# zyddnys/sd_animation_optical_flow

Hardware: AMD Instinct MI355X
Metric: frame-pairs/sec (flow+warp+mask) at 512x768 (higher is better)
Workload: dtype f32

## Files before the change

### sd_animation_optical_flow_amd/csrc/conv_wino.hip

```cpp
#include "ofx_internal.h"

#include <cmath>
#include <cstdlib>
#include <cstring>

namespace {

constexpr int kWBK = 16;
constexpr int kLDV = kWBK + 4;
constexpr int kOOB = 0x7FFFFFF0;

template <int W_, int H_, int LDH, int Y0, int X0> struct Halo {
    static constexpr int W = W_, H = H_, ldh = LDH, y_org = Y0, x_org = X0;
    static constexpr int pix = W * H;
    static constexpr int items = pix * (kWBK / 4);
    static constexpr int slots = (items + 255) / 256;
    static constexpr int floats = pix * ldh;
};
using Halo3x3 = Halo<18, 10, 24, -1, -1>;
template <bool VERT> using Halo15 = Halo<VERT ? 16 : 20, VERT ? 12 : 8, VERT ? 16 : 20, VERT ? -2 : 0, VERT ? 0 : -2>;

struct WinoK {
    const float* in0;
    const float* in1;
    const float* u;
    const float* scale;
    const float* shift;
    const float* addend;
    const float* res;
    const float* nmean;
    const float* nrstd;
    float* stats;
    float* out;
    float* aux_z;
    float* aux_rh;
    float* aux_h;
    int ld0, c0, ld1, cin, ldo, ldadd, ldh, ldres;
    int H, W, Cout, act;
    int nblk;
    int nb32;
    int tpr, tpi, mtiles;
    int bytes0, bytes1, bytesu;
    float alpha;
};

struct Patch {
    int nb, pb, y0, x0;
};

__device__ __forceinline__ Patch wino_patch(const WinoK& p) {
    const int nblk = p.mtiles * p.nblk;
    const int bid = blockIdx.x;
    const int q8 = nblk >> 3, r8 = nblk & 7;
    const int xcd = bid & 7, idx = bid >> 3;
    const int L = (xcd < r8 ? xcd * (q8 + 1) : r8 * (q8 + 1) + (xcd - r8) * q8) + idx;
    const int nb = L % p.nblk, mt = L / p.nblk;
    const int pb = mt / p.tpi;
    const int trem = mt - pb * p.tpi;
    const int py = trem / p.tpr;
    return {nb, pb, py * 8, (trem - py * p.tpr) * 16};
}

template <class ALG, bool NORM = false>
__device__ __forceinline__ void wino_slabs(const WinoK& p, const Patch& pt, float* Hs, float* Vs, int tid, int wave,
                                           f32x16 (&acc)[ALG::P][ALG::NT]) {
    typedef int v4i __attribute__((ext_vector_type(4)));
    using HALO = typename ALG::HALO;
    constexpr int P = ALG::P, NT = ALG::NT;
    const int lane = tid & 63;

    const float* in1s = p.in1 ? p.in1 : p.in0;
    const int bytes1s = p.in1 ? p.bytes1 : p.bytes0;
    int hpix[HALO::slots];
    unsigned hok = 0;
#pragma unroll
    for (int k = 0; k < HALO::slots; ++k) {
        const int i = tid + 256 * k;
        const int pix = i >> 2;
        const int hy = pix / HALO::W, hx = pix - hy * HALO::W;
        const int gy = pt.y0 + HALO::y_org + hy, gx = pt.x0 + HALO::x_org + hx;
        const bool ok = i < HALO::items && (unsigned)gy < (unsigned)p.H && (unsigned)gx < (unsigned)p.W;
        hpix[k] = ok ? (pt.pb * p.H + gy) * p.W + gx : 0;
        hok |= (ok ? 1u : 0u) << k;
    }
    const int hq = (tid & 3) * 16;
    float4 pa[HALO::slots];
    float4 pmu, prs;
    auto a_issue = [&](int cb) __attribute__((always_inline)) {
        const int c = cb * kWBK;
        const bool s0 = c < p.c0;
        const __amdgpu_buffer_rsrc_t rs = __builtin_amdgcn_make_buffer_rsrc((void*)(s0 ? p.in0 : in1s), (short)0, s0 ? p.bytes0 : bytes1s, 0x00020000);
        const int so = (s0 ? c : c - p.c0) * 4;
        const int ldb = (s0 ? p.ld0 : p.ld1) * 4;
#pragma unroll
        for (int k = 0; k < HALO::slots; ++k) {
            const int vo = ((hok >> k) & 1u) ? hpix[k] * ldb + hq : kOOB;
            v4i t = __builtin_amdgcn_raw_buffer_load_b128(rs, vo, so, 0);
            pa[k] = *reinterpret_cast<float4*>(&t);
        }
        if constexpr (NORM) {
            const long at = (long)pt.pb * p.c0 + c + (tid & 3) * 4;
            pmu = *reinterpret_cast<const float4*>(p.nmean + at);
            prs = *reinterpret_cast<const float4*>(p.nrstd + at);
        }
    };

    const __amdgpu_buffer_rsrc_t rsu = __builtin_amdgcn_make_buffer_rsrc((void*)p.u, (short)0, p.bytesu, 0x00020000);
    const int c8n = p.cin >> 3;
    const int wlane = lane * 16;
    const int pt0 = ALG::pt0(wave), blk0 = ALG::blk0(pt.nb, wave);
    float4 wr[P][NT][2];
    auto w_issue = [&](int q, int cb) __attribute__((always_inline)) {
#pragma unroll
        for (int nt = 0; nt < NT; ++nt)
#pragma unroll
            for (int ks = 0; ks < 2; ++ks) {
                const int so = (((pt0 + q) * p.nb32 + blk0 + nt) * c8n + 2 * cb + ks) * 1024;
                v4i t = __builtin_amdgcn_raw_buffer_load_b128(rsu, wlane, so, 0);
                wr[q][nt][ks] = *reinterpret_cast<float4*>(&t);
            }
    };

#pragma unroll
    for (int q = 0; q < P; ++q)
#pragma unroll
        for (int nt = 0; nt < NT; ++nt)
#pragma unroll
            for (int e = 0; e < 16; ++e) acc[q][nt][e] = 0.f;

    const ALG xf(Hs, Vs, tid, wave);
    const float* const afrag = Vs + (pt0 * 32 + (lane & 31)) * kLDV + 4 * (lane >> 5);

    const int CB = p.cin / kWBK;
    a_issue(0);
#pragma unroll
    for (int q = 0; q < P; ++q) w_issue(q, 0);
    for (int cb = 0; cb < CB; ++cb) {
        const int nx = cb + 1 < CB ? cb + 1 : cb;
#pragma unroll
        for (int k = 0; k < HALO::slots; ++k) {
            const int i = tid + 256 * k;
            if (HALO::slots * 256 > HALO::items && k == HALO::slots - 1 && i >= HALO::items) break;
            float4 v = pa[k];
            if constexpr (NORM) {
                v.x = fmaxf((v.x - pmu.x) * prs.x, 0.f);
                v.y = fmaxf((v.y - pmu.y) * prs.y, 0.f);
                v.z = fmaxf((v.z - pmu.z) * prs.z, 0.f);
                v.w = fmaxf((v.w - pmu.w) * prs.w, 0.f);
                if (!((hok >> k) & 1u)) v = make_float4(0.f, 0.f, 0.f, 0.f);
            }
            *reinterpret_cast<float4*>(&Hs[(i >> 2) * HALO::ldh + (i & 3) * 4]) = v;
        }
        __syncthreads();
        xf();
        __syncthreads();
        a_issue(nx);
        __builtin_amdgcn_sched_barrier(0);
#pragma unroll
        for (int q = 0; q < P; ++q) {
#pragma unroll
            for (int ks = 0; ks < 2; ++ks) {
                const float4 a = *reinterpret_cast<const float4*>(afrag + q * 32 * kLDV + 8 * ks);
#pragma unroll
                for (int nt = 0; nt < NT; ++nt) {
                    const float4 b = wr[q][nt][ks];
                    acc[q][nt] = __builtin_amdgcn_mfma_f32_32x32x2f32(a.x, b.x, acc[q][nt], 0, 0, 0);
                    acc[q][nt] = __builtin_amdgcn_mfma_f32_32x32x2f32(a.y, b.y, acc[q][nt], 0, 0, 0);
                    acc[q][nt] = __builtin_amdgcn_mfma_f32_32x32x2f32(a.z, b.z, acc[q][nt], 0, 0, 0);
                    acc[q][nt] = __builtin_amdgcn_mfma_f32_32x32x2f32(a.w, b.w, acc[q][nt], 0, 0, 0);
                }
            }
            w_issue(q, nx);
        }
    }
}

__device__ __forceinline__ float2 f2(float a, float b) { return make_float2(a, b); }
__device__ __forceinline__ float2 operator+(float2 a, float2 b) { return f2(a.x + b.x, a.y + b.y); }
__device__ __forceinline__ float2 operator-(float2 a, float2 b) { return f2(a.x - b.x, a.y - b.y); }
__device__ __forceinline__ float2 operator*(float s, float2 a) { return f2(s * a.x, s * a.y); }

struct Wino3x3 {
    using HALO = Halo3x3;
    static constexpr int P = 4, NT = 2;
    __device__ static int pt0(int wave) { return 4 * wave; }
    __device__ static int blk0(int nb, int) { return 2 * nb; }
    const float* src;
    float* dst;
    __device__ __forceinline__ Wino3x3(const float* Hs, float* Vs, int tid, int wave) {
        const int ttx = (tid & 63) >> 3, tcp = tid & 7;
        src = Hs + (2 * wave * HALO::W + 2 * ttx) * HALO::ldh + 2 * tcp;
        dst = Vs + (wave * 8 + ttx) * kLDV + 2 * tcp;
    }
    __device__ __forceinline__ void operator()() const {
        float2 d[4][4];
#pragma unroll
        for (int r = 0; r < 4; ++r)
#pragma unroll
            for (int c = 0; c < 4; ++c) d[r][c] = *reinterpret_cast<const float2*>(src + (r * HALO::W + c) * HALO::ldh);
        float2 t[4][4];
#pragma unroll
        for (int c = 0; c < 4; ++c) {
            t[0][c] = d[0][c] - d[2][c];
            t[1][c] = d[1][c] + d[2][c];
            t[2][c] = d[2][c] - d[1][c];
            t[3][c] = d[1][c] - d[3][c];
        }
#pragma unroll
        for (int i = 0; i < 4; ++i) {
            float2 v[4];
            v[0] = t[i][0] - t[i][2];
            v[1] = t[i][1] + t[i][2];
            v[2] = t[i][2] - t[i][1];
            v[3] = t[i][1] - t[i][3];
#pragma unroll
            for (int j = 0; j < 4; ++j) *reinterpret_cast<float2*>(dst + (i * 4 + j) * 32 * kLDV) = v[j];
        }
    }
};

template <bool VERT> struct Wino15 {
    using HALO = Halo15<VERT>;
    static constexpr int P = 8, NT = 1;
    __device__ static int pt0(int) { return 0; }
    __device__ static int blk0(int nb, int wave) { return 4 * nb + wave; }
    static constexpr int tap = (VERT ? HALO::W : 1) * HALO::ldh;
    const float* src;
    float* dst;
    __device__ static int base(int t) { return VERT ? (4 * (t >> 4)) * HALO::W + (t & 15) : (t >> 2) * HALO::W + 4 * (t & 3); }
    __device__ static int oy(int t, int i) { return VERT ? 4 * (t >> 4) + i : t >> 2; }
    __device__ static int ox(int t, int i) { return VERT ? (t & 15) : 4 * (t & 3) + i; }
    __device__ __forceinline__ Wino15(const float* Hs, float* Vs, int tid, int) {
        const int ttile = tid >> 3, tcp = tid & 7;
        src = Hs + base(ttile) * HALO::ldh + 2 * tcp;
        dst = Vs + ttile * kLDV + 2 * tcp;
    }
    __device__ __forceinline__ void operator()() const {
        float2 d[8];
#pragma unroll
        for (int j = 0; j < 8; ++j) d[j] = *reinterpret_cast<const float2*>(src + j * tap);
        float2 v[8];
        v[0] = (d[0] - d[6]) + 5.25f * (d[4] - d[2]);
        v[7] = (d[7] - d[1]) + 5.25f * (d[3] - d[5]);
        float2 te = (d[2] + d[6]) - 4.25f * d[4], to = (d[1] + d[5]) - 4.25f * d[3];
        v[1] = te + to;
        v[2] = te - to;
        te = (0.25f * d[2] + d[6]) - 1.25f * d[4];
        to = (0.5f * d[1] - 2.5f * d[3]) + 2.0f * d[5];
        v[3] = te + to;
        v[4] = te - to;
        te = (4.0f * d[2] + d[6]) - 5.0f * d[4];
        to = (2.0f * d[1] - 2.5f * d[3]) + 0.5f * d[5];
        v[5] = te + to;
        v[6] = te - to;
#pragma unroll
        for (int j = 0; j < 8; ++j) *reinterpret_cast<float2*>(dst + j * 32 * kLDV) = v[j];
    }
};

constexpr int kLDX = 32;
constexpr int kVF2 = 16 * 32 * kLDV;
constexpr int kSmem2 = Halo3x3::floats + kVF2;
constexpr int kXF = 4 * 2 * 32 * kLDX;
static_assert(kXF + 2 * 4 * 32 * 2 <= kSmem2, "exchange and statistics must fit");

template <bool NORM, bool RES, bool STATS>
__global__ __launch_bounds__(256, 2) void wino_conv_kernel(const WinoK p) {
    __shared__ __attribute__((aligned(16))) float smem[kSmem2];
    float* const Hs = smem;
    float* const Vs = smem + Halo3x3::floats;
    const int tid = threadIdx.x, lane = tid & 63;
    const int wave = __builtin_amdgcn_readfirstlane(tid >> 6);
    const Patch pt = wino_patch(p);
    f32x16 acc[4][2];
    wino_slabs<Wino3x3, NORM>(p, pt, Hs, Vs, tid, wave, acc);

    const float act_lo = p.act == OFX_ACT_RELU ? 0.0f : -3.402823466e38f;
    float* const X = smem;
    float* const Sx = smem + kXF;
    const int on = tid & 31, otx = tid >> 5;
#pragma unroll
    for (int nt = 0; nt < 2; ++nt) {
        __syncthreads();
#pragma unroll
        for (int e = 0; e < 16; ++e) {
            const int tile = (e & 3) + 8 * (e >> 2) + 4 * (lane >> 5);
            const float m0 = acc[0][nt][e], m1 = acc[1][nt][e], m2 = acc[2][nt][e], m3 = acc[3][nt][e];
            X[((wave * 2 + 0) * 32 + tile) * kLDX + (lane & 31)] = m0 + m1 + m2;
            X[((wave * 2 + 1) * 32 + tile) * kLDX + (lane & 31)] = m1 - m2 - m3;
        }
        __syncthreads();
        const int oc = pt.nb * 64 + nt * 32 + on;
        if (oc < p.Cout) {
            const float sc = (p.scale ? p.scale[oc] : 1.0f) * p.alpha;
            const float sh = p.shift ? p.shift[oc] : 0.0f;
            float st_s = 0.0f, st_q = 0.0f;
#pragma unroll
            for (int ty = 0; ty < 4; ++ty) {
                const int tile = ty * 8 + otx;
                float x[4][2];
#pragma unroll
                for (int w = 0; w < 4; ++w)
#pragma unroll
                    for (int j = 0; j < 2; ++j) x[w][j] = X[((w * 2 + j) * 32 + tile) * kLDX + on];
                float r[2][2];
                if constexpr (RES) {
#pragma unroll
                    for (int a = 0; a < 2; ++a)
#pragma unroll
                        for (int j = 0; j < 2; ++j)
                            r[a][j] = p.res[(((long)pt.pb * p.H + pt.y0 + 2 * ty + a) * p.W + pt.x0 + 2 * otx + j) * p.ldres + oc];
                }
#pragma unroll
                for (int a = 0; a < 2; ++a)
#pragma unroll
                    for (int j = 0; j < 2; ++j) {
                        const float y = a == 0 ? x[0][j] + x[1][j] + x[2][j] : x[1][j] - x[2][j] - x[3][j];
                        const long pix = ((long)pt.pb * p.H + pt.y0 + 2 * ty + a) * p.W + pt.x0 + 2 * otx + j;
                        float v = fmaxf(y * sc + sh, act_lo);
                        if constexpr (RES) v = fmaxf(v + r[a][j], 0.0f);
                        p.out[pix * p.ldo + oc] = v;
                        if constexpr (STATS) {
                            st_s += v;
                            st_q = fmaf(v, v, st_q);
                        }
                    }
            }
            if constexpr (STATS) {
                st_s += __shfl_xor(st_s, 32, 64);
                st_q += __shfl_xor(st_q, 32, 64);
                if (lane < 32) {
                    Sx[((nt * 4 + wave) * 32 + on) * 2 + 0] = st_s;
                    Sx[((nt * 4 + wave) * 32 + on) * 2 + 1] = st_q;
                }
            }
        }
    }
    if constexpr (STATS) {
        __syncthreads();
        const int nt = tid >> 5;
        const int oc = pt.nb * 64 + nt * 32 + on;
        if (tid < 64 && oc < p.Cout) {
            float s = 0.0f, q = 0.0f;
#pragma unroll
            for (int w = 0; w < 4; ++w) {
                s += Sx[((nt * 4 + w) * 32 + on) * 2 + 0];
                q += Sx[((nt * 4 + w) * 32 + on) * 2 + 1];
            }
            const long row = (long)pt.pb * p.tpi + (pt.y0 >> 3) * p.tpr + (pt.x0 >> 4);
            p.stats[(row * p.Cout + oc) * 2 + 0] = s;
            p.stats[(row * p.Cout + oc) * 2 + 1] = q;
        }
    }
}

int launch3x3(const WinoK& k, dim3 grid, dim3 block, hipStream_t s) {
    const int v = (k.nmean ? 4 : 0) | (k.res ? 2 : 0) | (k.stats ? 1 : 0);
    switch (v) {
        case 0: OFX_LAUNCH((wino_conv_kernel<false, false, false>), grid, block, s, k); break;
        case 1: OFX_LAUNCH((wino_conv_kernel<false, false, true>), grid, block, s, k); break;
        case 2: OFX_LAUNCH((wino_conv_kernel<false, true, false>), grid, block, s, k); break;
        case 4: OFX_LAUNCH((wino_conv_kernel<true, false, false>), grid, block, s, k); break;
        case 5: OFX_LAUNCH((wino_conv_kernel<true, false, true>), grid, block, s, k); break;
        case 6: OFX_LAUNCH((wino_conv_kernel<true, true, false>), grid, block, s, k); break;
        default: return OFX_EINVAL;
    }
    return ofx_launch_status();
}

template <bool VERT, int EPI>
__global__ __launch_bounds__(256, 2) void wino15_conv_kernel(const WinoK p) {
    using T = Wino15<VERT>;
    using HALO = typename T::HALO;
    __shared__ __attribute__((aligned(16))) float smem[HALO::floats + 8 * 32 * kLDV];
    float* const Hs = smem;
    float* const Vs = smem + HALO::floats;
    const int tid = threadIdx.x, lane = tid & 63;
    const int wave = __builtin_amdgcn_readfirstlane(tid >> 6);
    const Patch pt = wino_patch(p);
    f32x16 acc[8][1];
    wino_slabs<T>(p, pt, Hs, Vs, tid, wave, acc);

    const int n = pt.nb * 128 + wave * 32 + (lane & 31);
    if (n >= p.Cout) return;
    const float sc = (p.scale ? p.scale[n] : 1.0f) * p.alpha;
    const float sh = p.shift ? p.shift[n] : 0.0f;
    const float act_lo = p.act == OFX_ACT_RELU ? 0.0f : -3.402823466e38f;
    const int hd = p.Cout >> 1;
    const bool r_half = EPI == OFX_EPI_GRU_ZR && pt.nb * 128 >= hd;
#pragma unroll
    for (int eb = 0; eb < 16; eb += 4) {
        long pix[4][4];
        float y[4][4], ad[4][4], x1[4][4], x2[4][4];
#pragma unroll
        for (int u = 0; u < 4; ++u) {
            const int e = eb + u;
            const int tile = (e & 3) + 8 * (e >> 2) + 4 * (lane >> 5);
#pragma unroll
            for (int i = 0; i < 4; ++i) pix[u][i] = ((long)pt.pb * p.H + pt.y0 + T::oy(tile, i)) * p.W + pt.x0 + T::ox(tile, i);
            const float m0 = acc[0][0][e], m1 = acc[1][0][e], m2 = acc[2][0][e], m3 = acc[3][0][e];
            const float m4 = acc[4][0][e], m5 = acc[5][0][e], m6 = acc[6][0][e], m7 = acc[7][0][e];
            const float s12 = m1 + m2, d12 = m1 - m2, s34 = m3 + m4, d34 = m3 - m4, s56 = m5 + m6, d56 = m5 - m6;
            y[u][0] = m0 + s12 + s34 + s56;
            y[u][1] = d12 + 2.0f * d34 + 0.5f * d56;
            y[u][2] = s12 + 4.0f * s34 + 0.25f * s56;
            y[u][3] = d12 + 8.0f * d34 + 0.125f * d56 + m7;
        }
#pragma unroll
        for (int u = 0; u < 4; ++u)
#pragma unroll
            for (int i = 0; i < 4; ++i) {
                ad[u][i] = p.addend ? p.addend[pix[u][i] * p.ldadd + n] : 0.0f;
                x1[u][i] = EPI == OFX_EPI_GRU_ZR ? (r_half ? p.aux_h[pix[u][i] * p.ldh + n - hd] : 1.0f)
                           : EPI == OFX_EPI_GRU_Q ? p.aux_z[pix[u][i] * p.Cout + n] : 0.0f;
                x2[u][i] = EPI == OFX_EPI_GRU_Q ? p.aux_h[pix[u][i] * p.ldh + n] : 0.0f;
            }
#pragma unroll
        for (int u = 0; u < 4; ++u)
#pragma unroll
            for (int i = 0; i < 4; ++i) {
                const float v = y[u][i] * sc + sh + ad[u][i];
                if (EPI == OFX_EPI_PLAIN) {
                    p.out[pix[u][i] * p.ldo + n] = fmaxf(v, act_lo);
                } else if (EPI == OFX_EPI_GRU_ZR) {
                    const float g = ofx_sigmoid(v) * x1[u][i];
                    if (r_half) p.aux_rh[pix[u][i] * hd + n - hd] = g;
                    else p.aux_z[pix[u][i] * hd + n] = g;
                } else {
                    p.aux_h[pix[u][i] * p.ldh + n] = (1.0f - x1[u][i]) * x2[u][i] + x1[u][i] * ofx_tanh(v);
                }
            }
    }
}

template <bool VERT>
int launch15(const WinoK& k, int epi, dim3 grid, dim3 block, hipStream_t s) {
    switch (epi) {
        case OFX_EPI_PLAIN: OFX_LAUNCH((wino15_conv_kernel<VERT, OFX_EPI_PLAIN>), grid, block, s, k); break;
        case OFX_EPI_GRU_ZR: OFX_LAUNCH((wino15_conv_kernel<VERT, OFX_EPI_GRU_ZR>), grid, block, s, k); break;
        case OFX_EPI_GRU_Q: OFX_LAUNCH((wino15_conv_kernel<VERT, OFX_EPI_GRU_Q>), grid, block, s, k); break;
        default: return OFX_EINVAL;
    }
    return ofx_launch_status();
}

bool is_3x3(const ofx_conv_desc* d) { return d->KH == 3 && d->KW == 3; }
bool is_1d(int KH, int KW) { return (KH == 1 && KW == 5) || (KH == 5 && KW == 1); }
int wino_points(const ofx_conv_desc* d) { return is_3x3(d) ? 16 : 8; }
int wino_cblk(const ofx_conv_desc* d) { return is_3x3(d) ? 64 : 128; }

}

bool ofx_conv_wino_fits(const ofx_conv_desc* d) {
    const int cin = d->c0 + d->c1;
    const bool plain = d->epi == OFX_EPI_PLAIN && d->out != nullptr && d->ldo >= d->Cout && (d->act == OFX_ACT_NONE || d->act == OFX_ACT_RELU);
    bool shape_epi = false;
    if (is_3x3(d)) {
        shape_epi = d->padH == 1 && d->padW == 1 && plain && !d->addend && (!d->res || d->ldres >= d->Cout) &&
                    (!d->nmean || (d->nrstd && !d->in1 && ofx_aligned16(d->nmean) && ofx_aligned16(d->nrstd)));
    } else if (is_1d(d->KH, d->KW)) {
        shape_epi = d->padH == d->KH / 2 && d->padW == d->KW / 2 && !d->nmean && !d->res &&
                    (plain || (d->epi == OFX_EPI_GRU_ZR && (d->Cout / 2) % 128 == 0) || d->epi == OFX_EPI_GRU_Q);
    }
    return shape_epi && d->precision == OFX_PREC_FP32 && (d->nz <= 1) && d->stride == 1 && d->Hout == d->Hin && d->Wout == d->Win &&
           d->Hin % 8 == 0 && d->Win % 16 == 0 && cin % kWBK == 0 && d->c0 % kWBK == 0 &&
           d->wino_w != nullptr && ofx_aligned16(d->wino_w);
}

int ofx_conv_wino_stats_rows(const ofx_conv_desc* d) {
    return is_3x3(d) && d->act == OFX_ACT_NONE && !d->res ? (d->Hin / 8) * (d->Win / 16) : 0;
}

bool ofx_conv_wino_pays(const ofx_conv_desc* d) {
    const long patches = (long)d->B * (d->Hin / 8) * (d->Win / 16);
    return is_3x3(d) ? patches * ((d->Cout + 63) / 64) >= 1024 : patches >= 256;
}

double ofx_conv_wino_flops(const ofx_conv_desc* d) {
    return 2.0 * wino_points(d) * ((double)d->B * d->Hout * d->Wout / 4.0) * (double)(d->c0 + d->c1) * d->Cout;
}

int ofx_conv_wino_launch(const ofx_conv_desc* d, float alpha, float* stats, hipStream_t s) {
    OFX_REQUIRE(!stats || ofx_conv_wino_stats_rows(d) > 0, OFX_EINVAL);
    WinoK k;
    k.in0 = d->in0; k.in1 = d->in1; k.u = d->wino_w; k.scale = d->scale; k.shift = d->shift; k.addend = d->addend; k.out = d->out;
    k.res = d->res; k.nmean = d->nmean; k.nrstd = d->nrstd; k.stats = stats;
    k.aux_z = d->aux_z; k.aux_rh = d->aux_rh; k.aux_h = d->aux_h;
    k.ld0 = d->ld0; k.c0 = d->c0; k.ld1 = d->ld1; k.cin = d->c0 + d->c1; k.ldo = d->ldo; k.ldadd = d->ldadd; k.ldh = d->ldh;
    k.ldres = d->ldres;
    k.H = d->Hin; k.W = d->Win; k.Cout = d->Cout; k.act = d->act;
    const int cblk = wino_cblk(d);
    k.nblk = (d->Cout + cblk - 1) / cblk;
    k.nb32 = cblk / 32 * k.nblk;
    k.tpr = d->Win / 16;
    k.tpi = (d->Hin / 8) * k.tpr;
    const long mtiles = (long)d->B * k.tpi;
    const long npix = (long)d->B * d->Hin * d->Win;
    const long ext0 = ((npix - 1) * d->ld0 + d->c0) * 4, ext1 = d->in1 ? ((npix - 1) * d->ld1 + d->c1) * 4 : 0;
    const long extu = (long)wino_points(d) * k.nb32 * 32 * k.cin * 4;
    OFX_REQUIRE(ext0 < (1L << 31) - 64 && ext1 < (1L << 31) - 64 && extu < (1L << 31) - 64, OFX_EINVAL);
    OFX_REQUIRE(mtiles * k.nblk < (1L << 31) && (!is_3x3(d) || npix * d->ldo < (1L << 31)), OFX_EINVAL);
    k.mtiles = (int)mtiles;
    k.bytes0 = (int)ext0; k.bytes1 = (int)ext1; k.bytesu = (int)extu;
    k.alpha = alpha;
    const dim3 grid((unsigned)(k.mtiles * k.nblk), 1, 1), block(256, 1, 1);
    if (is_3x3(d)) return launch3x3(k, grid, block, s);
    return d->KH == 5 ? launch15<true>(k, d->epi, grid, block, s) : launch15<false>(k, d->epi, grid, block, s);
}

namespace {

template <class XF>
long wino_weight(const float* w, int Cout, int Cin, int taps, int points, int cblk, float* out, XF xf) {
    OFX_REQUIRE(Cout > 0 && Cin > 0 && Cin % kWBK == 0, OFX_EINVAL);
    const int nb32 = cblk / 32 * ((Cout + cblk - 1) / cblk);
    const long n = (long)points * nb32 * 32 * Cin;
    if (!out) return n;
    OFX_REQUIRE(w != nullptr, OFX_EINVAL);
    std::memset(out, 0, (size_t)n * sizeof(float));
    double u[16];
    for (int o = 0; o < Cout; ++o)
        for (int c = 0; c < Cin; ++c) {
            xf(w + ((size_t)o * Cin + c) * taps, u);
            for (int q = 0; q < points; ++q) {
                const long at = ((((long)q * nb32 + o / 32) * (Cin / 8) + c / 8) * 2 + (c % 8) / 4) * 128 + 4 * (o % 32) + c % 4;
                out[at] = (float)u[q];
            }
        }
    return n;
}

}

extern "C" long ofx_wino_conv_weight(const float* w, int Cout, int Cin, float* out) {
    return wino_weight(w, Cout, Cin, 9, 16, 64, out, [](const float* g, double* u) {
        static const double G[4][3] = {{1, 0, 0}, {0.5, 0.5, 0.5}, {0.5, -0.5, 0.5}, {0, 0, 1}};
        double gg[4][3];
        for (int i = 0; i < 4; ++i)
            for (int x = 0; x < 3; ++x) gg[i][x] = G[i][0] * g[x] + G[i][1] * g[3 + x] + G[i][2] * g[6 + x];
        for (int i = 0; i < 4; ++i)
            for (int j = 0; j < 4; ++j) u[4 * i + j] = gg[i][0] * G[j][0] + gg[i][1] * G[j][1] + gg[i][2] * G[j][2];
    });
}

extern "C" long ofx_wino15_conv_weight(const float* w, int Cout, int Cin, int KH, int KW, float* out) {
    OFX_REQUIRE(is_1d(KH, KW), OFX_EINVAL);
    return wino_weight(w, Cout, Cin, 5, 8, 128, out, [](const float* g, double* u) {
        static const double G[8][5] = {
            {1, 0, 0, 0, 0},
            {-2.0 / 9, -2.0 / 9, -2.0 / 9, -2.0 / 9, -2.0 / 9},
            {-2.0 / 9, 2.0 / 9, -2.0 / 9, 2.0 / 9, -2.0 / 9},
            {1.0 / 90, 1.0 / 45, 2.0 / 45, 4.0 / 45, 8.0 / 45},
            {1.0 / 90, -1.0 / 45, 2.0 / 45, -4.0 / 45, 8.0 / 45},
            {32.0 / 45, 16.0 / 45, 8.0 / 45, 4.0 / 45, 2.0 / 45},
            {32.0 / 45, -16.0 / 45, 8.0 / 45, -4.0 / 45, 2.0 / 45},
            {0, 0, 0, 0, 1},
        };
        for (int q = 0; q < 8; ++q) {
            u[q] = 0.0;
            for (int t = 0; t < 5; ++t) u[q] += G[q][t] * (double)g[t];
        }
    });
}
```

Baseline: 298.9.

## Fuse Winograd input transform into MFMA operand loads with double-buffered halo

The 3x3 Winograd kernel no longer writes transformed input tiles to a separate Vs buffer. Each wave now computes its rows of the B^T d B transform directly from a pair-interleaved halo layout in LDS, right before feeding the MFMAs. The halo is double-buffered so the next channel block is stored while the current one is consumed, which cuts one of the two barriers per iteration. Weight loads are now issued per 8-channel step, interleaved with the MFMAs. The trade-off is redundant transform arithmetic across waves, more LDS reads per MFMA, and a larger LDS footprint, which may affect occupancy.

```diff
diff --git a/sd_animation_optical_flow_amd/csrc/conv_wino.hip b/sd_animation_optical_flow_amd/csrc/conv_wino.hip
--- a/sd_animation_optical_flow_amd/csrc/conv_wino.hip
+++ b/sd_animation_optical_flow_amd/csrc/conv_wino.hip
@@ -10,15 +10,23 @@
 constexpr int kLDV = kWBK + 4;
 constexpr int kOOB = 0x7FFFFFF0;
 
-template <int W_, int H_, int LDH, int Y0, int X0> struct Halo {
-    static constexpr int W = W_, H = H_, ldh = LDH, y_org = Y0, x_org = X0;
+template <int W_, int H_, int Y0, int X0> struct HaloGeom {
+    static constexpr int W = W_, H = H_, y_org = Y0, x_org = X0;
     static constexpr int pix = W * H;
     static constexpr int items = pix * (kWBK / 4);
     static constexpr int slots = (items + 255) / 256;
-    static constexpr int floats = pix * ldh;
-};
-using Halo3x3 = Halo<18, 10, 24, -1, -1>;
-template <bool VERT> using Halo15 = Halo<VERT ? 16 : 20, VERT ? 12 : 8, VERT ? 16 : 20, VERT ? -2 : 0, VERT ? 0 : -2>;
+};
+template <bool VERT> struct Halo15 : HaloGeom<VERT ? 16 : 20, VERT ? 12 : 8, VERT ? -2 : 0, VERT ? 0 : -2> {
+    static constexpr int ldh = VERT ? 16 : 20;
+    static constexpr int floats = Halo15::pix * ldh;
+    __device__ static int at(int pix) { return pix * ldh; }
+};
+struct Halo3x3 : HaloGeom<18, 10, -1, -1> {
+    static constexpr int lpair = 36, lrow = 336;
+    static constexpr int floats = H * lrow;
+    __device__ static int at(int y, int x) { return y * lrow + (x >> 1) * lpair + (x & 1) * 16; }
+    __device__ static int at(int pix) { return at(pix / W, pix % W); }
+};
 
 struct WinoK {
     const float* in0;
@@ -61,32 +69,35 @@
     return {nb, pb, py * 8, (trem - py * p.tpr) * 16};
 }
 
-template <class ALG, bool NORM = false>
-__device__ __forceinline__ void wino_slabs(const WinoK& p, const Patch& pt, float* Hs, float* Vs, int tid, int wave,
-                                           f32x16 (&acc)[ALG::P][ALG::NT]) {
-    typedef int v4i __attribute__((ext_vector_type(4)));
-    using HALO = typename ALG::HALO;
-    constexpr int P = ALG::P, NT = ALG::NT;
-    const int lane = tid & 63;
-
-    const float* in1s = p.in1 ? p.in1 : p.in0;
-    const int bytes1s = p.in1 ? p.bytes1 : p.bytes0;
+typedef int v4i __attribute__((ext_vector_type(4)));
+
+template <class HALO, bool NORM> struct HaloStage {
+    const WinoK& p;
+    const int pb, tid;
+    const float* in1s;
+    int bytes1s;
     int hpix[HALO::slots];
     unsigned hok = 0;
-#pragma unroll
-    for (int k = 0; k < HALO::slots; ++k) {
-        const int i = tid + 256 * k;
-        const int pix = i >> 2;
-        const int hy = pix / HALO::W, hx = pix - hy * HALO::W;
-        const int gy = pt.y0 + HALO::y_org + hy, gx = pt.x0 + HALO::x_org + hx;
-        const bool ok = i < HALO::items && (unsigned)gy < (unsigned)p.H && (unsigned)gx < (unsigned)p.W;
-        hpix[k] = ok ? (pt.pb * p.H + gy) * p.W + gx : 0;
-        hok |= (ok ? 1u : 0u) << k;
-    }
-    const int hq = (tid & 3) * 16;
+    int hq;
     float4 pa[HALO::slots];
     float4 pmu, prs;
-    auto a_issue = [&](int cb) __attribute__((always_inline)) {
+
+    __device__ __forceinline__ HaloStage(const WinoK& p_, const Patch& pt, int tid_) : p(p_), pb(pt.pb), tid(tid_) {
+        in1s = p.in1 ? p.in1 : p.in0;
+        bytes1s = p.in1 ? p.bytes1 : p.bytes0;
+#pragma unroll
+        for (int k = 0; k < HALO::slots; ++k) {
+            const int i = tid + 256 * k;
+            const int pix = i >> 2;
+            const int hy = pix / HALO::W, hx = pix - hy * HALO::W;
+            const int gy = pt.y0 + HALO::y_org + hy, gx = pt.x0 + HALO::x_org + hx;
+            const bool ok = i < HALO::items && (unsigned)gy < (unsigned)p.H && (unsigned)gx < (unsigned)p.W;
+            hpix[k] = ok ? (pt.pb * p.H + gy) * p.W + gx : 0;
+            hok |= (ok ? 1u : 0u) << k;
+        }
+        hq = (tid & 3) * 16;
+    }
+    __device__ __forceinline__ void issue(int cb) {
         const int c = cb * kWBK;
         const bool s0 = c < p.c0;
         const __amdgpu_buffer_rsrc_t rs = __builtin_amdgcn_make_buffer_rsrc((void*)(s0 ? p.in0 : in1s), (short)0, s0 ? p.bytes0 : bytes1s, 0x00020000);
@@ -99,44 +110,12 @@
             pa[k] = *reinterpret_cast<float4*>(&t);
         }
         if constexpr (NORM) {
-            const long at = (long)pt.pb * p.c0 + c + (tid & 3) * 4;
+            const long at = (long)pb * p.c0 + c + (tid & 3) * 4;
             pmu = *reinterpret_cast<const float4*>(p.nmean + at);
             prs = *reinterpret_cast<const float4*>(p.nrstd + at);
         }
-    };
-
-    const __amdgpu_buffer_rsrc_t rsu = __builtin_amdgcn_make_buffer_rsrc((void*)p.u, (short)0, p.bytesu, 0x00020000);
-    const int c8n = p.cin >> 3;
-    const int wlane = lane * 16;
-    const int pt0 = ALG::pt0(wave), blk0 = ALG::blk0(pt.nb, wave);
-    float4 wr[P][NT][2];
-    auto w_issue = [&](int q, int cb) __attribute__((always_inline)) {
-#pragma unroll
-        for (int nt = 0; nt < NT; ++nt)
-#pragma unroll
-            for (int ks = 0; ks < 2; ++ks) {
-                const int so = (((pt0 + q) * p.nb32 + blk0 + nt) * c8n + 2 * cb + ks) * 1024;
-                v4i t = __builtin_amdgcn_raw_buffer_load_b128(rsu, wlane, so, 0);
-                wr[q][nt][ks] = *reinterpret_cast<float4*>(&t);
-            }
-    };
-
-#pragma unroll
-    for (int q = 0; q < P; ++q)
-#pragma unroll
-        for (int nt = 0; nt < NT; ++nt)
-#pragma unroll
-            for (int e = 0; e < 16; ++e) acc[q][nt][e] = 0.f;
-
-    const ALG xf(Hs, Vs, tid, wave);
-    const float* const afrag = Vs + (pt0 * 32 + (lane & 31)) * kLDV + 4 * (lane >> 5);
-
-    const int CB = p.cin / kWBK;
-    a_issue(0);
-#pragma unroll
-    for (int q = 0; q < P; ++q) w_issue(q, 0);
-    for (int cb = 0; cb < CB; ++cb) {
-        const int nx = cb + 1 < CB ? cb + 1 : cb;
+    }
+    __device__ __forceinline__ void store(float* Hs) const {
 #pragma unroll
         for (int k = 0; k < HALO::slots; ++k) {
             const int i = tid + 256 * k;
@@ -149,7 +128,114 @@
                 v.w = fmaxf((v.w - pmu.w) * prs.w, 0.f);
                 if (!((hok >> k) & 1u)) v = make_float4(0.f, 0.f, 0.f, 0.f);
             }
-            *reinterpret_cast<float4*>(&Hs[(i >> 2) * HALO::ldh + (i & 3) * 4]) = v;
+            *reinterpret_cast<float4*>(&Hs[HALO::at(i >> 2) + (i & 3) * 4]) = v;
+        }
+    }
+};
+
+struct WinoU {
+    const __amdgpu_buffer_rsrc_t rs;
+    const int nb32, c8n, wlane;
+    __device__ __forceinline__ WinoU(const WinoK& p, int lane)
+        : rs(__builtin_amdgcn_make_buffer_rsrc((void*)p.u, (short)0, p.bytesu, 0x00020000)), nb32(p.nb32), c8n(p.cin >> 3), wlane(lane * 16) {}
+    __device__ __forceinline__ float4 load(int pt, int blk, int c8) const {
+        const int so = ((pt * nb32 + blk) * c8n + c8) * 1024;
+        v4i t = __builtin_amdgcn_raw_buffer_load_b128(rs, wlane, so, 0);
+        return *reinterpret_cast<float4*>(&t);
+    }
+};
+
+template <int P, int NT> __device__ __forceinline__ void wino_zero(f32x16 (&acc)[P][NT]) {
+#pragma unroll
+    for (int q = 0; q < P; ++q)
+#pragma unroll
+        for (int nt = 0; nt < NT; ++nt)
+#pragma unroll
+            for (int e = 0; e < 16; ++e) acc[q][nt][e] = 0.f;
+}
+
+__device__ __forceinline__ void wino_mfma4(f32x16& acc, const float4& a, const float4& b) {
+    acc = __builtin_amdgcn_mfma_f32_32x32x2f32(a.x, b.x, acc, 0, 0, 0);
+    acc = __builtin_amdgcn_mfma_f32_32x32x2f32(a.y, b.y, acc, 0, 0, 0);
+    acc = __builtin_amdgcn_mfma_f32_32x32x2f32(a.z, b.z, acc, 0, 0, 0);
+    acc = __builtin_amdgcn_mfma_f32_32x32x2f32(a.w, b.w, acc, 0, 0, 0);
+}
+
+template <class ALG>
+__device__ __forceinline__ void wino_slabs_staged(const WinoK& p, const Patch& pt, float* Hs, float* Vs, int tid, int wave,
+                                           f32x16 (&acc)[ALG::P][ALG::NT]) {
+    using HALO = typename ALG::HALO;
+    constexpr int P = ALG::P, NT = ALG::NT;
+    const int lane = tid & 63;
+
+    const float* in1s = p.in1 ? p.in1 : p.in0;
+    const int bytes1s = p.in1 ? p.bytes1 : p.bytes0;
+    int hpix[HALO::slots];
+    unsigned hok = 0;
+#pragma unroll
+    for (int k = 0; k < HALO::slots; ++k) {
+        const int i = tid + 256 * k;
+        const int pix = i >> 2;
+        const int hy = pix / HALO::W, hx = pix - hy * HALO::W;
+        const int gy = pt.y0 + HALO::y_org + hy, gx = pt.x0 + HALO::x_org + hx;
+        const bool ok = i < HALO::items && (unsigned)gy < (unsigned)p.H && (unsigned)gx < (unsigned)p.W;
+        hpix[k] = ok ? (pt.pb * p.H + gy) * p.W + gx : 0;
+        hok |= (ok ? 1u : 0u) << k;
+    }
+    const int hq = (tid & 3) * 16;
+    float4 pa[HALO::slots];
+    auto a_issue = [&](int cb) __attribute__((always_inline)) {
+        const int c = cb * kWBK;
+        const bool s0 = c < p.c0;
+        const __amdgpu_buffer_rsrc_t rs = __builtin_amdgcn_make_buffer_rsrc((void*)(s0 ? p.in0 : in1s), (short)0, s0 ? p.bytes0 : bytes1s, 0x00020000);
+        const int so = (s0 ? c : c - p.c0) * 4;
+        const int ldb = (s0 ? p.ld0 : p.ld1) * 4;
+#pragma unroll
+        for (int k = 0; k < HALO::slots; ++k) {
+            const int vo = ((hok >> k) & 1u) ? hpix[k] * ldb + hq : kOOB;
+            v4i t = __builtin_amdgcn_raw_buffer_load_b128(rs, vo, so, 0);
+            pa[k] = *reinterpret_cast<float4*>(&t);
+        }
+    };
+
+    const __amdgpu_buffer_rsrc_t rsu = __builtin_amdgcn_make_buffer_rsrc((void*)p.u, (short)0, p.bytesu, 0x00020000);
+    const int c8n = p.cin >> 3;
+    const int wlane = lane * 16;
+    const int pt0 = ALG::pt0(wave), blk0 = ALG::blk0(pt.nb, wave);
+    float4 wr[P][NT][2];
+    auto w_issue = [&](int q, int cb) __attribute__((always_inline)) {
+#pragma unroll
+        for (int nt = 0; nt < NT; ++nt)
+#pragma unroll
+            for (int ks = 0; ks < 2; ++ks) {
+                const int so = (((pt0 + q) * p.nb32 + blk0 + nt) * c8n + 2 * cb + ks) * 1024;
+                v4i t = __builtin_amdgcn_raw_buffer_load_b128(rsu, wlane, so, 0);
+                wr[q][nt][ks] = *reinterpret_cast<float4*>(&t);
+            }
+    };
+
+#pragma unroll
+    for (int q = 0; q < P; ++q)
+#pragma unroll
+        for (int nt = 0; nt < NT; ++nt)
+#pragma unroll
+            for (int e = 0; e < 16; ++e) acc[q][nt][e] = 0.f;
+
+    const ALG xf(Hs, Vs, tid, wave);
+    const float* const afrag = Vs + (pt0 * 32 + (lane & 31)) * kLDV + 4 * (lane >> 5);
+
+    const int CB = p.cin / kWBK;
+    a_issue(0);
+#pragma unroll
+    for (int q = 0; q < P; ++q) w_issue(q, 0);
+    for (int cb = 0; cb < CB; ++cb) {
+        const int nx = cb + 1 < CB ? cb + 1 : cb;
+#pragma unroll
+        for (int k = 0; k < HALO::slots; ++k) {
+            const int i = tid + 256 * k;
+            if (HALO::slots * 256 > HALO::items && k == HALO::slots - 1 && i >= HALO::items) break;
+            float4 v = pa[k];
+            *reinterpret_cast<float4*>(&Hs[HALO::at(i >> 2) + (i & 3) * 4]) = v;
         }
         __syncthreads();
         xf();
@@ -175,49 +261,66 @@
     }
 }
 
+__device__ __forceinline__ float4 operator+(float4 a, float4 b) { return make_float4(a.x + b.x, a.y + b.y, a.z + b.z, a.w + b.w); }
+__device__ __forceinline__ float4 operator-(float4 a, float4 b) { return make_float4(a.x - b.x, a.y - b.y, a.z - b.z, a.w - b.w); }
+
+template <bool NORM>
+__device__ __forceinline__ void wino3x3_slabs(const WinoK& p, const Patch& pt, float* Hs, int tid, int wave, f32x16 (&acc)[4][2]) {
+    using HALO = Halo3x3;
+    const int lane = tid & 63;
+    HaloStage<HALO, NORM> hs(p, pt, tid);
+    const WinoU u(p, lane);
+    const int pt0 = 4 * wave, blk0 = 2 * pt.nb;
+    float4 wr[4][2];
+    wino_zero(acc);
+
+    const int ra = wave == 0 ? 0 : wave == 2 ? 2 : 1, rb = wave == 2 ? 1 : wave == 3 ? 3 : 2;
+    const float sg = wave == 1 ? 1.0f : -1.0f;
+    const int tile = lane & 31;
+    const int at0 = HALO::at(2 * (tile >> 3), 2 * (tile & 7)) + 4 * (lane >> 5);
+    const int at_a = at0 + ra * HALO::lrow, at_b = at0 + rb * HALO::lrow;
+
+    const int CB = p.cin / kWBK;
+    hs.issue(0);
+#pragma unroll
+    for (int q = 0; q < 4; ++q)
+#pragma unroll
+        for (int nt = 0; nt < 2; ++nt) wr[q][nt] = u.load(pt0 + q, blk0 + nt, 0);
+    hs.store(Hs);
+    hs.issue(CB > 1 ? 1 : 0);
+    for (int cb = 0; cb < CB; ++cb) {
+        const float* const H = Hs + (cb & 1) * HALO::floats;
+        __syncthreads();
+        hs.store(Hs + (~cb & 1) * HALO::floats);
+        hs.issue(cb + 2 < CB ? cb + 2 : CB - 1);
+        __builtin_amdgcn_sched_barrier(0);
+#pragma unroll
+        for (int ks = 0; ks < 2; ++ks) {
+            float4 t[4];
+#pragma unroll
+            for (int c = 0; c < 4; ++c) {
+                const float4 a = *reinterpret_cast<const float4*>(H + at_a + HALO::at(0, c) + 8 * ks);
+                const float4 b = *reinterpret_cast<const float4*>(H + at_b + HALO::at(0, c) + 8 * ks);
+                t[c] = make_float4(__builtin_fmaf(sg, b.x, a.x), __builtin_fmaf(sg, b.y, a.y), __builtin_fmaf(sg, b.z, a.z),
+                                   __builtin_fmaf(sg, b.w, a.w));
+            }
+            const float4 v[4] = {t[0] - t[2], t[1] + t[2], t[2] - t[1], t[1] - t[3]};
+            const int c8 = 2 * cb + ks + 1 < 2 * CB ? 2 * cb + ks + 1 : 2 * cb + ks;
+#pragma unroll
+            for (int q = 0; q < 4; ++q)
+#pragma unroll
+                for (int nt = 0; nt < 2; ++nt) {
+                    wino_mfma4(acc[q][nt], v[q], wr[q][nt]);
+                    wr[q][nt] = u.load(pt0 + q, blk0 + nt, c8);
+                }
+        }
+    }
+}
+
 __device__ __forceinline__ float2 f2(float a, float b) { return make_float2(a, b); }
 __device__ __forceinline__ float2 operator+(float2 a, float2 b) { return f2(a.x + b.x, a.y + b.y); }
 __device__ __forceinline__ float2 operator-(float2 a, float2 b) { return f2(a.x - b.x, a.y - b.y); }
 __device__ __forceinline__ float2 operator*(float s, float2 a) { return f2(s * a.x, s * a.y); }
-
-struct Wino3x3 {
-    using HALO = Halo3x3;
-    static constexpr int P = 4, NT = 2;
-    __device__ static int pt0(int wave) { return 4 * wave; }
-    __device__ static int blk0(int nb, int) { return 2 * nb; }
-    const float* src;
-    float* dst;
-    __device__ __forceinline__ Wino3x3(const float* Hs, float* Vs, int tid, int wave) {
-        const int ttx = (tid & 63) >> 3, tcp = tid & 7;
-        src = Hs + (2 * wave * HALO::W + 2 * ttx) * HALO::ldh + 2 * tcp;
-        dst = Vs + (wave * 8 + ttx) * kLDV + 2 * tcp;
-    }
-    __device__ __forceinline__ void operator()() const {
-        float2 d[4][4];
-#pragma unroll
-        for (int r = 0; r < 4; ++r)
-#pragma unroll
-            for (int c = 0; c < 4; ++c) d[r][c] = *reinterpret_cast<const float2*>(src + (r * HALO::W + c) * HALO::ldh);
-        float2 t[4][4];
-#pragma unroll
-        for (int c = 0; c < 4; ++c) {
-            t[0][c] = d[0][c] - d[2][c];
-            t[1][c] = d[1][c] + d[2][c];
-            t[2][c] = d[2][c] - d[1][c];
-            t[3][c] = d[1][c] - d[3][c];
-        }
-#pragma unroll
-        for (int i = 0; i < 4; ++i) {
-            float2 v[4];
-            v[0] = t[i][0] - t[i][2];
-            v[1] = t[i][1] + t[i][2];
-            v[2] = t[i][2] - t[i][1];
-            v[3] = t[i][1] - t[i][3];
-#pragma unroll
-            for (int j = 0; j < 4; ++j) *reinterpret_cast<float2*>(dst + (i * 4 + j) * 32 * kLDV) = v[j];
-        }
-    }
-};
 
 template <bool VERT> struct Wino15 {
     using HALO = Halo15<VERT>;
@@ -259,21 +362,18 @@
 };
 
 constexpr int kLDX = 32;
-constexpr int kVF2 = 16 * 32 * kLDV;
-constexpr int kSmem2 = Halo3x3::floats + kVF2;
 constexpr int kXF = 4 * 2 * 32 * kLDX;
-static_assert(kXF + 2 * 4 * 32 * 2 <= kSmem2, "exchange and statistics must fit");
+constexpr int kSX = 2 * 4 * 32 * 2;
+constexpr int kSmem2 = 2 * Halo3x3::floats > kXF + kSX ? 2 * Halo3x3::floats : kXF + kSX;
 
 template <bool NORM, bool RES, bool STATS>
 __global__ __launch_bounds__(256, 2) void wino_conv_kernel(const WinoK p) {
     __shared__ __attribute__((aligned(16))) float smem[kSmem2];
-    float* const Hs = smem;
-    float* const Vs = smem + Halo3x3::floats;
     const int tid = threadIdx.x, lane = tid & 63;
     const int wave = __builtin_amdgcn_readfirstlane(tid >> 6);
     const Patch pt = wino_patch(p);
     f32x16 acc[4][2];
-    wino_slabs<Wino3x3, NORM>(p, pt, Hs, Vs, tid, wave, acc);
+    wino3x3_slabs<NORM>(p, pt, smem, tid, wave, acc);
 
     const float act_lo = p.act == OFX_ACT_RELU ? 0.0f : -3.402823466e38f;
     float* const X = smem;
@@ -379,7 +479,7 @@
     const int wave = __builtin_amdgcn_readfirstlane(tid >> 6);
     const Patch pt = wino_patch(p);
     f32x16 acc[8][1];
-    wino_slabs<T>(p, pt, Hs, Vs, tid, wave, acc);
+    wino_slabs_staged<T>(p, pt, Hs, Vs, tid, wave, acc);
 
     const int n = pt.nb * 128 + wave * 32 + (lane & 31);
     if (n >= p.Cout) return;
```

After: 303.2 (median of 6 runs). 1.4% higher.
